# ysong1231/SimRank

Measured on AMD Instinct MI355X. Metric: simrank_iterations_per_sec, higher is better.
Workload: dtype f32

## Files before the change

simrank_amd/csrc/api.hip:

```cpp
#include <algorithm>
#include <chrono>
#include <cstring>
#include <mutex>
#include <unordered_map>
#include <string>
#include <thread>
#include <vector>

#include "common.h"

namespace simrank {

static thread_local char g_err[512] = "";

void set_error(const char* fmt, ...) {
    va_list ap;
    va_start(ap, fmt);
    vsnprintf(g_err, sizeof(g_err), fmt, ap);
    va_end(ap);
}

Tuning& tuning() {
    static Tuning t;
    return t;
// ... 67 lines not shown
            l.push_back((int32_t)rt);
        }
    }
    size_t longest = 0;
    for (const auto& l : lists) longest = std::max(longest, l.size() / 2);
    sym_map.assign(longest * 8 * 2, -1);
    for (size_t x = 0; x < 8; ++x)
        for (size_t k = 0; k < lists[x].size() / 2; ++k) {
            sym_map[2 * (8 * k + x)] = lists[x][2 * k];
            sym_map[2 * (8 * k + x) + 1] = lists[x][2 * k + 1];
        }
    return n_tiles;
}

void build_short_image(const int32_t* rowptr, const int32_t* col, const float* rowscale, int64_t n_rows,
                       const std::vector<int32_t>& tile_row0, int64_t n_tiles, int32_t width, ShortImage& out) {
    out = ShortImage();
    if ((width != 8 && width != 16) || n_tiles <= 0 || n_rows < 64) return;
    const int64_t groups = (n_tiles + 3) / 4;
    out.is_short.assign((size_t)groups, 0);
    for (int64_t k = 0; k < groups; ++k) {
        bool ok = true;
        for (int64_t t = 4 * k; ok && t < std::min<int64_t>(4 * k + 4, n_tiles); ++t) {
            const int64_t lo = tile_row0[(size_t)t], hi = tile_row0[(size_t)t + 1];
            ok = lo % 32 == 0 && hi == std::min<int64_t>(n_rows, lo + 32);
            for (int64_t a = lo; ok && a < hi; ++a) ok = rowptr[a + 1] - rowptr[a] <= width;
        }
        out.is_short[(size_t)k] = ok ? 1 : 0;
        out.groups += ok ? 1 : 0;
    }
    if (out.groups == 0) return;
    out.width = width;
    const size_t tiles_pad = (size_t)groups * 4;
    out.tiles.assign(tiles_pad * 2, 0);
    out.meta.assign(tiles_pad * 8 * 8, 0u);
    out.ids.assign(tiles_pad * 64 * (size_t)(width / 2), (uint16_t)0xFFFF);
    const int nc = width / 8;
    for (int64_t t = 0; t < n_tiles; ++t) {
        if (!out.is_short[(size_t)(t / 4)]) continue;
        const int32_t lo = tile_row0[(size_t)t];
        const int nrows = tile_row0[(size_t)t + 1] - lo;
        out.tiles[2 * (size_t)t] = lo;
        out.tiles[2 * (size_t)t + 1] = nrows;
        int order[32];
        for (int r = 0; r < nrows; ++r) order[r] = r;
        std::sort(order, order + nrows, [&](int x, int y) {
            const int32_t lx = rowptr[lo + x + 1] - rowptr[lo + x], ly = rowptr[lo + y + 1] - rowptr[lo + y];
            return lx != ly ? lx > ly : x > y;
        });
        for (int s = 0; s < nrows; ++s) {
            const int r = order[s], ps = s / 8, g = s % 8;
            const int32_t start = rowptr[lo + r], len = rowptr[lo + r + 1] - start;
            uint32_t* m = out.meta.data() + ((size_t)t * 8 + (size_t)g) * 8;
            std::memcpy(m + ps, rowscale + lo + r, 4);
            m[4] |= (uint32_t)len << (8 * ps);
            m[5] |= (uint32_t)r << (8 * ps);
            for (int32_t j = 0; j < len; ++j) {
                const int lane = 8 * g + (j & 7), c = j >> 3;
                out.ids[((size_t)t * 64 + (size_t)lane) * (size_t)(width / 2) + (size_t)(ps * nc + c)] = (uint16_t)col[start + j];
            }
        }
    }
}

namespace {
constexpr size_t kPoolMin = size_t(64) << 20;
constexpr size_t kSmallLimit = size_t(1) << 30;
constexpr int kSmallClasses = 4 * 40;
inline size_t small_class_bytes(int c) { return (size_t(4 + (c & 3)) << (c >> 2)) * 128; }
inline int small_class_of(size_t bytes) {
    int c = 0;
    while (small_class_bytes(c) < bytes) ++c;
    return c;
}
// ... 614 lines not shown
    int rc = up((void**)&g->rowptr, rowptr, size_t(n_rows + 1) * 4);
    if (!rc) rc = up((void**)&g->col, col, size_t(nnz) * 4);
    if (!rc && n_cols <= 65536 && nnz > 0) {
        std::vector<uint16_t> c16(col, col + nnz);
        rc = up((void**)&g->col16, c16.data(), size_t(nnz) * 2);
    }
    if (!rc) rc = up((void**)&g->rowscale, rowscale, size_t(n_rows) * 4);
    if (!rc) rc = up((void**)&g->t_rowptr, t_rowptr.data(), size_t(n_cols + 1) * 4);
    if (!rc) rc = up((void**)&g->t_col, t_col.data(), size_t(nnz) * 4);
    if (!rc) rc = up((void**)&g->t_pos, t_pos.data(), size_t(nnz) * 4);
    if (!rc && g->ev_hubs) rc = up((void**)&g->ev_hubidx, hubidx.data(), size_t(n_cols) * 4);
    if (!rc && g->n_tiles) rc = up((void**)&g->tile_row0, tile_row0.data(), tile_row0.size() * 4);
    if (!rc && g->sym_blocks) rc = up((void**)&g->sym_map, sym_map.data(), sym_map.size() * 4);
    if (!rc && g->sym_blocks && g->col16 && g->tun.leg2_short > 0) {
        ShortImage img;
        build_short_image(rowptr, col, rowscale, n_rows, tile_row0, g->n_tiles, (int32_t)g->tun.leg2_short, img);
        if (img.groups > 0) {
            for (size_t k = 0; k < sym_map.size() / 2; ++k)
                if (sym_map[2 * k] >= 0 && img.is_short[(size_t)sym_map[2 * k + 1]]) sym_map[2 * k + 1] |= 1 << 30;
            g->short_w = img.width;
            g->short_groups = img.groups;
            rc = up((void**)&g->sym_map_short, sym_map.data(), sym_map.size() * 4);
            if (!rc) rc = up((void**)&g->short_tiles, img.tiles.data(), img.tiles.size() * 4);
            if (!rc) rc = up((void**)&g->short_meta, img.meta.data(), img.meta.size() * 4);
            if (!rc) rc = up((void**)&g->short_ids, img.ids.data(), img.ids.size() * 2);
        }
    }
    if (!rc && after_base && *after_base) rc = (*after_base)(g);
    const double t_base = since();
    for (int i = 0; i < n_jobs; ++i) {
        jobs[i].th.join();
        if (timed) std::fprintf(stderr, "simrank_graph_create: builder %d took %.1f ms\n", i, jobs[i].ms);
        if (!rc && jobs[i].rc) {
            rc = jobs[i].rc;
// ... 172 lines not shown
        t.fuse_dens = value;
    } else if (!strcmp(key, "dense_cols")) {
        SR_REQUIRE(value >= 1 && value <= (1 << 20), "dense_cols must be >= 1");
        t.dense_cols = value;
    } else if (!strcmp(key, "restrict_support")) {
        SR_REQUIRE(value >= -1 && value <= 1, "restrict_support must be -1 (automatic), 0 or 1");
        t.restrict_support = value;
    } else if (!strcmp(key, "leg1_skip")) {
        t.leg1_skip = value ? 1 : 0;
    } else if (!strcmp(key, "leg1_order")) {
        SR_REQUIRE(value >= -1 && value <= 1, "leg1_order must be -1 (by the graph's size), 0 or 1");
        t.leg1_order = value;
    } else if (!strcmp(key, "leg2_short")) {
        SR_REQUIRE(value == 0 || value == 8 || value == 16, "leg2_short must be 0 (off), 8 or 16");
        t.leg2_short = value;
    } else {
        SR_REQUIRE(false, "unknown tuning key '%s'", key);
    }
    return SIMRANK_OK;
}

int simrank_get_tuning(const char* key, int64_t* value) {
    SR_REQUIRE(key && value, "NULL argument");
    const Tuning t = tuning_snapshot();
    if (!strcmp(key, "panel")) *value = t.panel;
    else if (!strcmp(key, "xcd_map")) *value = t.xcd_map;
    else if (!strcmp(key, "stream_nt")) *value = t.stream_nt;
    else if (!strcmp(key, "tile")) *value = t.tile;
    else if (!strcmp(key, "triangle")) *value = t.triangle;
    else if (!strcmp(key, "huge")) *value = t.huge;
// ... 18 lines not shown
    else if (!strcmp(key, "fuse_max_rows")) *value = t.fuse_max_rows;
    else if (!strcmp(key, "fuse_order")) *value = t.fuse_order;
    else if (!strcmp(key, "fuse_store")) *value = t.fuse_store;
    else if (!strcmp(key, "fuse_meta_nt")) *value = t.fuse_meta_nt;
    else if (!strcmp(key, "sym_desc")) *value = t.sym_desc;
    else if (!strcmp(key, "ids16")) *value = t.ids16;
    else if (!strcmp(key, "lean")) *value = t.lean;
    else if (!strcmp(key, "addr32")) *value = t.addr32;
    else if (!strcmp(key, "probe_flags")) *value = t.probe_flags;
    else if (!strcmp(key, "dense_terms")) *value = t.dense_terms;
    else if (!strcmp(key, "probe_mask")) *value = t.probe_mask;
    else if (!strcmp(key, "restrict_support")) *value = t.restrict_support;
    else if (!strcmp(key, "leg1_skip")) *value = t.leg1_skip;
    else if (!strcmp(key, "leg1_order")) *value = t.leg1_order;
    else if (!strcmp(key, "leg2_short")) *value = t.leg2_short;
    else SR_REQUIRE(false, "unknown tuning key '%s'", key);
    return SIMRANK_OK;
}

int simrank_graph_get(const simrank_graph* g, const char* key, int64_t* value) {
    SR_REQUIRE(g && key && value, "NULL argument");
    if (!strcmp(key, "fused_ids16")) *value = g->fused ? g->fused->ids16 : -1;
    else if (!strcmp(key, "gather_ids16")) *value = (g->col16 && g->tun.ids16) ? 1 : 0;
    else if (!strcmp(key, "leg2_short_groups")) *value = g->short_groups;
    else if (!strcmp(key, "leg2_short_taken")) *value = g->leg2_short_taken;
    else if (!strcmp(key, "ev_hubs")) *value = g->ev_hub_cols;
    else SR_REQUIRE(false, "unknown graph key '%s'", key);
    return SIMRANK_OK;
}

}
```

simrank_amd/csrc/biplan.hip:

```cpp
#include <algorithm>
#include <cstring>
#include <numeric>
#include <vector>

#include <chrono>
#include <string>
#include <thread>

#include "loop.h"
#include "side.h"

using simrank::side_t;

struct simrank_biplan {
    side_t s[2];
    unsigned long long* counters = nullptr;
    unsigned long long* host_counters[2][2] = {{nullptr, nullptr}, {nullptr, nullptr}};
    hipEvent_t counted[2] = {nullptr, nullptr};
    hipStream_t stream = nullptr;
    int32_t updates = 0;
    int32_t broadcast_error = 0;
    int32_t asym = 0;
    int32_t identity_leg1 = 1;
    int32_t at_identity = 0;
// ... 82 lines not shown
        if (rc) return rc;
    }
    lap("validated, ordered, both patterns renamed");
    const float* priors[2] = {opt->apriori1, opt->apriori2};
    const int64_t lds[2] = {opt->ld_apriori1, opt->ld_apriori2};
    const int64_t ns[2] = {n1, n2};
    const std::vector<int32_t>* ord = pp.ord;
    const std::vector<int32_t>* inv = pp.inv;
    simrank_biplan* p = new simrank_biplan;
    p->stream = as_stream(stream);
    p->asym = pp.asym ? 1 : 0;
    if (const char* e = std::getenv("SIMRANK_IDENTITY_LEG1")) p->identity_leg1 = (*e == '0') ? 0 : 1;
    auto fail = [&](int code) { simrank_biplan_destroy(p); return code; };
    {
        Tuning tw[2] = {tuning_snapshot(), Tuning()};
        tw[1] = tw[0];
        int rcs[2] = {SIMRANK_OK, SIMRANK_OK};
        std::string errs[2];
        for (int w = 0; w < 2; ++w) {
            side_t& a = p->s[w];
            side_shape(a, ns[w], ns[w ^ 1], false);
            a.coef = w == 0 ? opt->c1 : opt->c2;
            a.lbd = w == 0 ? opt->lbd1 : opt->lbd2;
            if (tw[w].fuse == 1 && ((tw[w].triangle && a.n >= 64) || p->asym) && a.k <= tw[w].fuse_max_rows &&
                (a.k_rows_pad + 1) * 128 < (int64_t(1) << 31))
                tw[w].dense_lazy = 1;
        }
        auto make = [&](int w) {
            side_t& a = p->s[w];
            rcs[w] = graph_create_with(tw[w], a.n, a.k, nnz, pp.rp[w].data(), pp.cl[w].data(), pp.rs[w].data(), &a.g);
// ... 182 lines not shown
```

simrank_amd/csrc/common.h:

```cpp
#pragma once
#include <hip/hip_runtime.h>

#include <cstdarg>
#include <atomic>
#include <cstdint>
#include <cstdio>
#include <cstdlib>
#include <cstring>
#include <functional>
#include <vector>

#include "simrank_hip.h"

namespace simrank {

void set_error(const char* fmt, ...);

#define SR_HIP(call)                                                                   \
    do {                                                                               \
        hipError_t e_ = (call);                                                        \
        if (e_ != hipSuccess) {                                                        \
            ::simrank::set_error("%s failed: %s (%s:%d)", #call, hipGetErrorString(e_), \
                                 __FILE__, __LINE__);                                  \
            return SIMRANK_ERR_HIP;                                                    \
// ... 14 lines not shown
    int64_t stream_nt = 1;
    int64_t tile = 0;
    int64_t huge = 512;
    int64_t triangle = 1;
    int64_t balance = 2;
    int64_t dense_min = 4;
    int64_t dense_cols = 128;
    int64_t dense_terms = 3;
    int64_t probe_mask = -1;
    int64_t probe_flags = 0;
    int64_t addr32 = 1;
    int64_t lean = 1;
    int64_t ids16 = 1;
    int64_t sym_desc = 1;
    int64_t leg2_short = 16;
    int64_t ev_tri = 1;
    int64_t ev_hub = 14;
    int64_t fuse = 1;
    int64_t fuse_min = 0;
    int64_t fuse_pays = -1;
    int64_t fuse_steps = -1;
    int64_t fuse_dens = 0;
    int64_t fuse_unit = 48;
    int64_t fuse_rows = 8192;
    int64_t fuse_store = 1;
    int64_t fuse_meta_nt = 0;
    int64_t fuse_order = 0;
    int64_t fuse_max_rows = 1 << 20;
    int64_t fuse_cap = 40000;
    int64_t fuse_wgs = 4;
// ... 188 lines not shown
#endif
struct DenseUse {
    const float* part = nullptr;
    int64_t ldp = 0;
    const int32_t* block_slab0 = nullptr;
    const int32_t* block_nslab = nullptr;
};
void free_dense_plan(simrank_dense_plan* p);
int build_dense_plan(simrank_graph* g, const int32_t* rowptr, const int32_t* col);
int launch_dense_tiles(const simrank_graph* g, const float* X, int64_t ldx, int64_t L, bool tri,
                       hipStream_t st, DenseUse* use);
int64_t build_tiles(const int32_t* rowptr, int64_t n_rows, int64_t nnz, int64_t balance,
                    std::vector<int32_t>& tile_row0, std::vector<int32_t>& sym_map, bool sym_descending);
struct ShortImage {
    int32_t width = 0, groups = 0;
    std::vector<uint8_t> is_short;
    std::vector<int32_t> tiles;
    std::vector<uint32_t> meta;
    std::vector<uint16_t> ids;
};
void build_short_image(const int32_t* rowptr, const int32_t* col, const float* rowscale, int64_t n_rows,
                       const std::vector<int32_t>& tile_row0, int64_t n_tiles, int32_t width, ShortImage& out);
}

struct simrank_graph {
    int64_t n_rows = 0, n_cols = 0, nnz = 0;
    int32_t* rowptr = nullptr;
    int32_t* col = nullptr;
    uint16_t* col16 = nullptr;
    float* rowscale = nullptr;
    int32_t* t_rowptr = nullptr;
    int32_t* t_col = nullptr;
    int32_t* t_pos = nullptr;
    int32_t* ev_hubidx = nullptr;
    int32_t ev_hubs = 0;
    int32_t ev_hub_cols = 0;
    uint8_t* ev_hub_image = nullptr;
    void* ev_hub_ready = nullptr;
    int32_t max_row_nnz = 0;
    int32_t* tile_row0 = nullptr;
    int32_t n_tiles = 0;
    int32_t* sym_map = nullptr;
    int32_t sym_blocks = 0;
    int32_t* sym_map_short = nullptr;
    uint32_t* short_ids = nullptr;
    uint32_t* short_meta = nullptr;
    int32_t* short_tiles = nullptr;
    int32_t short_w = 0, short_groups = 0;
    mutable int32_t leg2_short_taken = 0;
    simrank_dense_plan* dense = nullptr;
    simrank_fused_plan* fused = nullptr;
    std::atomic<int> fused_build{0};
#ifdef SIMRANK_EXPERIMENT_FUSED2
    simrank_fused2_plan* fused2 = nullptr;
#endif
    simrank::Tuning tun;
};
```

simrank_amd/csrc/shardplan.hip:

```cpp
#include <dlfcn.h>
#include <rccl/rccl.h>

#include <algorithm>
#include <chrono>
#include <condition_variable>
#include <cstdlib>
#include <cstring>
#include <deque>
#include <mutex>
#include <vector>

#include "common.h"
#include "loop.h"

static_assert(sizeof(ncclUniqueId) == SIMRANK_COMM_ID_BYTES, "RCCL's unique id is SIMRANK_COMM_ID_BYTES long");

namespace simrank {

struct Rccl {
    void* lib = nullptr;
    ncclResult_t (*GetUniqueId)(ncclUniqueId*) = nullptr;
    ncclResult_t (*CommInitRank)(ncclComm_t*, int, ncclUniqueId, int) = nullptr;
    ncclResult_t (*CommDestroy)(ncclComm_t) = nullptr;
    ncclResult_t (*GroupStart)() = nullptr;
// ... 876 lines not shown
    }
    p->ld = pitch(p->Lm, 4);
    p->ld_ev = pitch(p->Lm, 1);
    p->pad = row_pad(p->mb);
    p->send_ld = int64_t(P) * (p->mb + p->pad);
    p->recv_ld = std::max<int64_t>(1, p->Lm + p->pad);
    p->n_stages = in.stages > 0 ? in.stages : int32_t(std::max<int64_t>(1, std::min<int64_t>(4, ((k + P - 1) / P) / 2048)));
    p->ord = ord;
    auto fail = [&](int code) { simrank_shardplan_destroy(p); return code; };
    p->half = fp16 ? 1 : 0;
    p->rows_pad = (n + 7) / 8 * 8 + 8;
    p->rows_pad_t = (p->Lm + 7) / 8 * 8 + 8;
    int rc;
    {
        Tuning t = tuning_snapshot();
        if (fp16) t.fuse_unit = int64_t(1) << 20;
        rc = graph_create_with(t, n, k, in.nnz, in.pat->rp->data(), in.pat->cl->data(), in.pat->rs->data(), &p->g);
    }
    if (rc) return fail(rc);
    if (fp16 && !p->g->fused) {
        set_error("storage_fp16 needs the one-launch plan (tuning fuse = 1) and a graph that has one");
        return fail(SIMRANK_ERR_INVALID);
    }
#define SP_HIP(call)                                                                              \
    do {                                                                                          \
        hipError_t e_ = (call);                                                                   \
        if (e_ != hipSuccess) {                                                                   \
            set_error("%s failed: %s (%s:%d)", #call, hipGetErrorString(e_), __FILE__, __LINE__); \
            (void)hipGetLastError();                                                              \
            return fail(e_ == hipErrorOutOfMemory ? SIMRANK_ERR_ALLOC : SIMRANK_ERR_HIP);         \
// ... 708 lines not shown
```

simrank_amd/csrc/side.h:

```cpp
#pragma once
#include <cstring>
#include <vector>

#include "common.h"

namespace simrank {

constexpr float kHalfScale = 16384.0f;

#define SIDE_HIP(call)                                                                            \
    do {                                                                                          \
        hipError_t e_ = (call);                                                                   \
        if (e_ != hipSuccess) {                                                                   \
            set_error("%s failed: %s (%s:%d)", #call, hipGetErrorString(e_), __FILE__, __LINE__); \
            (void)hipGetLastError();                                                              \
            return e_ == hipErrorOutOfMemory ? SIMRANK_ERR_ALLOC : SIMRANK_ERR_HIP;               \
        }                                                                                         \
    } while (0)

struct side_t {
    int64_t n = 0, k = 0, rows_pad = 0, k_rows_pad = 0;
    size_t mat_bytes = 0, t_bytes = 0;
    simrank_graph* g = nullptr;
    float* S[2] = {nullptr, nullptr};
    float* Tt = nullptr;
    uint8_t* ev = nullptr;
    float* prior = nullptr;
    int32_t* inv = nullptr;
    int32_t* ord_dev = nullptr;
    std::vector<int32_t> ord;
    float coef = 0.8f, lbd = 0.f;
    int32_t restrict_support = 0;
    int32_t half = 0;
    int cur = 0;
    int32_t* first_block = nullptr;
    std::vector<int32_t> first_block_host;
    int64_t leg1_units = 0, leg1_skipped = 0;
    int64_t leg2_short_groups = 0;
    int64_t dead_units = -1;
};

inline size_t side_f32_bytes(const side_t& a) { return size_t((a.n + 31) / 32) * size_t(a.rows_pad) * 32 * sizeof(float); }

inline void side_shape(side_t& a, int64_t n, int64_t k, bool half) {
    a.n = n;
    a.k = k;
    a.half = half ? 1 : 0;
    a.rows_pad = (n + 7) / 8 * 8 + 8;
    a.k_rows_pad = (k + 7) / 8 * 8 + 8;
    const size_t panels = half ? size_t((n + 63) / 64) : size_t((n + 31) / 32);
    a.mat_bytes = panels * size_t(a.rows_pad) * 128;
    a.t_bytes = panels * size_t(a.k_rows_pad) * 128;
}
// ... 112 lines not shown
            a.leg1_skipped = a.dead_units;
        }
    }
    if (!rc) rc = stamp();
    if (rc) return rc;
    if (asym) {
        ep.symmetric = 0;
        ep.restrict_support = 0;
        rc = simrank_spmm_blocked(a.g, a.Tt, a.k_rows_pad, a.n, a.S[nx], a.rows_pad, 1, nullptr, st);
        if (!rc) rc = simrank_epilogue_apply_blocked(a.S[nx], a.S[nx], a.n, a.n, a.rows_pad, &ep, st);
    } else {
        rc = a.half ? simrank_spmm_blocked_h16(a.g, a.Tt, a.k_rows_pad, a.n, a.S[nx], a.rows_pad, 0, &ep, a.rows_pad, kHalfScale, st)
                    : simrank_spmm_blocked(a.g, a.Tt, a.k_rows_pad, a.n, a.S[nx], a.rows_pad, 0, &ep, st);
    }
    a.leg2_short_groups = (asym || a.half || rc) ? 0 : a.g->leg2_short_taken;
    if (!rc) rc = stamp();
    if (rc) return rc;
    SR_HIP(hipMemcpyAsync(host_slot, counters, sizeof(unsigned long long) * SIMRANK_CHANGED_SLOTS, hipMemcpyDeviceToHost, st));
    return SIMRANK_OK;
}

inline int side_f32(const side_t& a, hipStream_t st, const float** src, float** scratch) {
    *src = a.S[a.cur];
    *scratch = nullptr;
    if (!a.half) return SIMRANK_OK;
    SR_HIP(pool_hip_alloc((void**)scratch, side_f32_bytes(a)));
    *src = *scratch;
    return simrank_widen_blocked_h16(a.S[a.cur], a.rows_pad, *scratch, a.rows_pad, a.n, a.n, kHalfScale, st);
}

// ... 68 lines not shown
    }
    return SIMRANK_OK;
}

inline int side_get(const side_t& a, const char* key, int64_t* value) {
    if (!strcmp(key, "restrict_support")) *value = a.restrict_support;
    else if (!strcmp(key, "iterate")) *value = (int64_t)(uintptr_t)a.S[a.cur];
    else if (!strcmp(key, "iterate_layout")) *value = a.half ? 2 : 0;
    else if (!strcmp(key, "iterate_stride")) *value = a.rows_pad;
    else if (!strcmp(key, "iterate_rows") || !strcmp(key, "iterate_col_hi")) *value = a.n;
    else if (!strcmp(key, "iterate_col_lo")) *value = 0;
    else if (!strcmp(key, "ids")) *value = (int64_t)(uintptr_t)a.ord_dev;
    else if (!strcmp(key, "leg1_units")) *value = a.leg1_units;
    else if (!strcmp(key, "leg1_skipped")) *value = a.leg1_skipped;
    else if (!strcmp(key, "leg2_short_groups")) *value = a.leg2_short_groups;
    else if (!strcmp(key, "graph")) *value = (int64_t)(uintptr_t)a.g;
    else SR_REQUIRE(false, "unknown plan key '%s'", key);
    return SIMRANK_OK;
}

}
```

simrank_amd/csrc/spmm.hip:

```cpp
#include <algorithm>
#include <type_traits>

#include <mutex>

#include "common.h"

namespace simrank {

__device__ __forceinline__ int64_t imin(int64_t a, int64_t b) { return a < b ? a : b; }

__device__ __forceinline__ int64_t elem_at(int64_t r, int64_t c, int64_t ld, int64_t rows_pad) {
    return rows_pad ? ((c >> 5) * rows_pad + r) * 32 + (c & 31) : r * ld + c;
}

struct SpmmArgs {
    const int32_t* rowptr;
    const int32_t* col;
    const uint16_t* col16;
    int32_t blocked;
    int64_t x_rows_pad, y_rows_pad;
    int64_t x_span_bytes;
    int32_t x_sentinel;
    int32_t addr32;
    int32_t sh_rank, sh_mb;
// ... 38 lines not shown
    int64_t ld_ev;
    const float* ap;
    int64_t ld_ap;
    const float* prev;
    int64_t ld_prev;
    double eps;
    unsigned long long* n_changed;
    int64_t diag_col0;
    int32_t set_diag;
    int32_t count_any;
    int32_t restrict_support;
    const float* dpart;
    int64_t ldp;
    const int32_t* dslab0;
    const int32_t* dnslab;
};

template <int VEC>
__device__ __forceinline__ void vload(float (&d)[VEC], const float* p) {
    if constexpr (VEC == 4) {
        const float4 t = *reinterpret_cast<const float4*>(p);
        d[0] = t.x; d[1] = t.y; d[2] = t.z; d[3] = t.w;
    } else {
        d[0] = *p;
    }
}

template <int VEC>
__device__ __forceinline__ void vstore(float* p, const float (&d)[VEC]) {
    if constexpr (VEC == 4) {
// ... 651 lines not shown
                for (int i = 0; i < 4; ++i) t[i * (RT + 1)] = o[i];
            }
        }
        float* y = p.Y + a * p.ldy + colofs;
        if (p.probe & 2) {
        } else if (nvalid == 4) {
            if (p.nt) vstore_nt<4>(y, o); else vstore<4>(y, o);
        } else {
#pragma unroll
            for (int i = 0; i < 4; ++i)
                if (i < nvalid) y[i] = o[i];
        }
    }
}

constexpr int kShortFlag = 1 << 30;

__device__ __forceinline__ void short_group3(const SpmmArgs& p, const Src32& xs, float* tbuf_wave, int t, int panel, int lane,
                                             int64_t c0, int64_t mycol, int64_t colofs, bool col_active, bool check_prev,
                                             unsigned& changed) {
    constexpr int RT = 32, PW = 32;
    typedef unsigned v2u __attribute__((ext_vector_type(2)));
    typedef unsigned v4u __attribute__((ext_vector_type(4)));
    typedef float f4 __attribute__((ext_vector_type(4)));
    const int g = lane >> 3, q = lane & 7, gbase = lane & ~7;
    const int nc = p.short_w >> 3;
    const int row0 = p.short_tiles[2 * t];
    int nrows = p.short_tiles[2 * t + 1];
    const uint32_t* idp = p.short_ids + (size_t(t) * 64 + lane) * size_t(2 * nc);
    v4u idw = {0u, 0u, 0u, 0u};
    if (nc == 2) {
        idw = *reinterpret_cast<const v4u*>(idp);
    } else {
        const v2u w = *reinterpret_cast<const v2u*>(idp);
        idw.x = w.x;
        idw.y = w.y;
    }
    const uint32_t* meta = p.short_meta + (size_t(t) * 8 + g) * 8;
    const f4 scales = *reinterpret_cast<const f4*>(meta);
    const v2u lr = *reinterpret_cast<const v2u*>(meta + 4);
    if (row0 > c0) nrows = 0;
    const bool mirror = row0 < c0;
    if (nrows == 0) return;

    const __amdgpu_buffer_rsrc_t prd = __builtin_amdgcn_make_buffer_rsrc(
        const_cast<float*>(check_prev ? p.prev + int64_t(panel) * p.y_rows_pad * 32 : p.prev), 0,
        check_prev ? int(p.y_rows_pad * 128) : 0, 0x00020000);
    float old[4][4];
#pragma unroll
    for (int ps = 0; ps < 4; ++ps) {
        const int r = int((lr.y >> (8 * ps)) & 255u);
        const v4u w = __builtin_amdgcn_raw_buffer_load_b128(prd, (row0 + r) * 128 + q * 16, 0, 2);
        old[ps][0] = __uint_as_float(w.x); old[ps][1] = __uint_as_float(w.y);
        old[ps][2] = __uint_as_float(w.z); old[ps][3] = __uint_as_float(w.w);
    }
    const float dsum[4] = {0.f, 0.f, 0.f, 0.f};
    auto pass = [&](int ps, const float (&old_ps)[4], float sc) {
        if (8 * ps >= nrows) return;
        const int len = int((lr.x >> (8 * ps)) & 255u);
        const int r = int((lr.y >> (8 * ps)) & 255u);
        const int n = (p.probe & 1) ? 0 : __builtin_amdgcn_readfirstlane(len);
        float acc[4] = {0.f, 0.f, 0.f, 0.f};
#pragma unroll 1
        for (int k = 0; k < n; k += 8) {
            const int h = ps * nc + (k >> 3);
            const unsigned w01 = (h & 2) ? idw.y : idw.x, w23 = (h & 2) ? idw.w : idw.z;
            const int raw = int((((h & 4) ? w23 : w01) >> (16 * (h & 1))) & 0xFFFFu);
            const int iv = (k + q < len && !(p.probe & 8)) ? (raw & p.idx_mask) : xs.sent();
            gather_chunk<1>(xs, iv, gbase, min(8, n - k), 0, 0, acc);
        }
        if (8 * ps + g < nrows && col_active)
            emit_row3<kSym>(p, tbuf_wave, r, int64_t(row0) + r, q, mycol, colofs, sc, acc, dsum, changed, mirror, check_prev, old_ps);
    };
    pass(0, old[0], scales.x);
    pass(1, old[1], scales.y);
    pass(2, old[2], scales.z);
    pass(3, old[3], scales.w);

    if (mirror && !(p.probe & 2)) {
        __builtin_amdgcn_fence(__ATOMIC_RELEASE, "wavefront");
        __builtin_amdgcn_wave_barrier();
        __builtin_amdgcn_fence(__ATOMIC_ACQUIRE, "wavefront");
        const int cols_here = int(imin(PW, p.L - c0));
        float* base = p.Y + ((int64_t(row0 >> 5) * p.y_rows_pad) + c0) * 32;
        if (cols_here == PW && (nrows & 3) == 0) {
#pragma unroll
            for (int it = 0; it < PW * (RT / 4) / 64; ++it) {
                const int x = lane + it * 64;
                const int c = x >> 3;
                const int r4 = (x & 7) * 4;
                if (r4 < nrows) {
                    const float* tb = tbuf_wave + c * (RT + 1) + r4;
                    const float v4[4] = {tb[0], tb[1], tb[2], tb[3]};
                    float* dst = base + c * 32 + r4;
                    if (p.nt) vstore_nt<4>(dst, v4); else vstore<4>(dst, v4);
                }
            }
        } else {
            for (int x = lane; x < PW * RT; x += 64) {
                const int c = x >> 5;
                const int r = x & 31;
                if (c < cols_here && r < nrows) base[c * 32 + r] = tbuf_wave[c * (RT + 1) + r];
            }
        }
    }
}

#ifdef SIMRANK_STAMPS
__device__ unsigned long long g_stamps[16];
__device__ __forceinline__ unsigned long long stamp_now() {
    unsigned long long t;
    __builtin_amdgcn_sched_barrier(0);
    asm volatile("s_memtime %0\n\ts_waitcnt lgkmcnt(0)" : "=s"(t) :: "memory");
    __builtin_amdgcn_sched_barrier(0);
    return t;
}
#define STAMP(i)                                                          \
    do {                                                                  \
        const unsigned long long now_ = stamp_now();                      \
        if (lane == 0) atomicAdd(&g_stamps[i], now_ - stamp_prev);        \
        stamp_prev = now_;                                                \
    } while (0)
#else
#define STAMP(i) do {} while (0)
#endif

template <int MODE, bool IDS16, bool RESTRICT, bool DENSE, bool A32, bool SHORT = false>
#ifndef SIMRANK_LB_DELTA
#define SIMRANK_LB_DELTA 0
#endif
__global__ __launch_bounds__(256, (MODE == kTrans ? ((DENSE && !A32) ? 7 : 8) : (DENSE ? 5 : 6)) - SIMRANK_LB_DELTA)
void gather3_kernel(const SpmmArgs p) {
    constexpr bool TRANS = MODE == kTrans;
    constexpr bool TILE = MODE != kPlain;
    constexpr int PW = 32, RT = 32, LPR = 8;
    extern __shared__ __attribute__((aligned(16))) float smem[];
    if (p.probe & 32) return;

    const int lane = threadIdx.x & 63;
    const int wave = __builtin_amdgcn_readfirstlane(threadIdx.x >> 6);
#ifdef SIMRANK_STAMPS
    unsigned long long stamp_prev = stamp_now();
// ... 66 lines not shown
    const unsigned slot = ((blockIdx.x * 4u + unsigned(wave)) * 7u) % SIMRANK_CHANGED_SLOTS;
    if constexpr (!TRANS) {
        {
            typedef unsigned v2u __attribute__((ext_vector_type(2)));
            const bool watch = p.has_ep && p.prev && p.count_any;
            const __amdgpu_buffer_rsrc_t csrd = __builtin_amdgcn_make_buffer_rsrc(
                const_cast<unsigned long long*>(p.n_changed), 0, watch ? SIMRANK_CHANGED_SLOTS * 8 : 0, 0x00020000);
            const v2u w = __builtin_amdgcn_raw_buffer_load_b64(csrd, int(slot * 8u), 0, 16);
            seen = (unsigned long long)w.x | ((unsigned long long)w.y << 32);
        }
    }

    if constexpr (SHORT) {
        if (rt & kShortFlag) {
            const bool cp = p.has_ep && p.prev && __builtin_amdgcn_readfirstlane(int(seen != 0)) == 0;
            const int t = (rt & ~kShortFlag) * kWaves + wave;
            short_group3(p, xs, tbuf_wave, t, panel, lane, c0, mycol, colofs, col_active, cp, changed);
            STAMP(3);
            if (p.has_ep && p.prev) {
#pragma unroll
                for (int off = 32; off > 0; off >>= 1) changed += __shfl_down(changed, off);
                if (lane == 0 && changed) atomicAdd(p.n_changed + slot, (unsigned long long)changed);
            }
            return;
        }
    }

    int row0 = (rt * kWaves + wave) * RT;
    int nrows = int(imin(RT, p.M - row0));
    if (p.tile_row0) {
        const int t = rt * kWaves + wave;
        const int tc = __builtin_amdgcn_readfirstlane(max(0, min(t, p.n_tiles - 1)));
// ... 304 lines not shown
            }
        }
    }

    STAMP(5);
    if constexpr (!TRANS) {
        if (p.has_ep && p.prev) {
#pragma unroll
            for (int off = 32; off > 0; off >>= 1) changed += __shfl_down(changed, off);
            if (lane == 0 && changed) atomicAdd(p.n_changed + slot, (unsigned long long)changed);
        }
    }
}

template <int MODE>
static int launch_gather3(SpmmArgs a, hipStream_t st, int32_t* short_taken = nullptr) {
    constexpr int PW = 32, RT = 32;
    a.n_panels = int((a.L + PW - 1) / PW);
    if (MODE == kShard && a.sh_ntiles > 0) a.n_panels = a.sh_ntiles;
    const int64_t rows_per_block = int64_t(kWaves) * RT;
    a.row_tiles = int((a.M + rows_per_block - 1) / rows_per_block);
    if (MODE == kSym && !a.sym_map) a.tile_row0 = nullptr;
    if (a.tile_row0) a.row_tiles = (a.n_tiles + kWaves - 1) / kWaves;
    const int64_t panels_padded = a.xcd_map ? int64_t((a.n_panels + 7) / 8) * 8 : a.n_panels;
    int64_t grid = panels_padded * a.row_tiles;
    if constexpr (MODE == kSym) {
        const int64_t J = (a.n_panels + 7) / 8;
        grid = 8 * (J * J + J);
        if (a.tile_row0) grid = a.sym_blocks;
    }
    SR_REQUIRE(grid > 0 && grid < (int64_t(1) << 31), "grid of %lld blocks", (long long)grid);
    const size_t lds = sizeof(float) * ((MODE != kPlain ? size_t(kWaves) * PW * (RT + 1) : 0) +
                                        (a.has_huge ? 64 + size_t(kMaxHuge) * kWaves * PW : 0));
    const bool restricted = MODE != kTrans && a.has_ep && a.ev && a.restrict_support;
    const bool dense = a.dpart != nullptr;
    const dim3 gr((unsigned)grid), bl(256);
    const int64_t x_rows = a.blocked ? a.x_rows_pad : a.K;
    const int64_t span = a.blocked ? a.x_rows_pad * 128 : ((x_rows - 1) * a.ldx + a.ldx) * 4;
    const bool a32 = a.addr32 && (x_rows + 1) * a.ldx * 4 + 256 < (int64_t(1) << 31) &&
                     a.ldx * 4 < (int64_t(1) << 24) && x_rows < (int64_t(1) << 24) - 1;
    a.x_span_bytes = span;
    a.x_sentinel = (int32_t)x_rows;
    const bool take_short = MODE == kSym && a.sym_map_short && a.short_groups > 0 && a.tile_row0 && a32 && a.col16 &&
                            !restricted && !dense && a.blocked;
    if (!take_short) a.short_groups = 0;
    if (short_taken) *short_taken = a.short_groups;
    if constexpr (MODE == kSym) {
        if (take_short) {
            a.sym_map = a.sym_map_short;
            hipLaunchKernelGGL((gather3_kernel<kSym, true, false, false, true, true>), gr, bl, lds, st, a);
            SR_HIP(hipGetLastError());
            return SIMRANK_OK;
        }
    }
#define SR_LAUNCH3(IDS, RES, DEN) \
    do { if (a32) hipLaunchKernelGGL((gather3_kernel<MODE, IDS, RES, DEN, true>), gr, bl, lds, st, a); \
         else hipLaunchKernelGGL((gather3_kernel<MODE, IDS, RES, DEN, false>), gr, bl, lds, st, a); } while (0)
#define SR_LAUNCH3_IDS(RES, DEN) \
    do { if (a.col16) SR_LAUNCH3(true, RES, DEN); else SR_LAUNCH3(false, RES, DEN); } while (0)
    if constexpr (MODE != kTrans) {
        if (restricted) {
            if (dense) SR_LAUNCH3_IDS(true, true); else SR_LAUNCH3_IDS(true, false);
// ... 615 lines not shown
    a.M = g->n_rows;
    a.K = g->n_cols;
    a.tblock = (t_block <= 0 || t_block > g->n_rows) ? g->n_rows : t_block;
    a.tstride = (transpose_out && a.tblock == g->n_rows && ldy >= g->n_rows) ? ldy : 0;
    a.tpad = a.tstride ? 0 : t_pad;
    a.tvec = aligned16(Y) && (a.tstride ? a.tstride % 4 == 0
                                        : (a.tblock % 4 == 0 && a.tpad % 4 == 0 && g->n_rows % 4 == 0));
    a.xcd_map = (int)T.xcd_map;
    a.idx_mask = (int32_t)T.probe_mask;
    a.addr32 = (int32_t)T.addr32;
    a.probe = (int32_t)T.probe_flags;
    bool vec_ok = aligned16(X) && ldx % 4 == 0;
    if (!transpose_out) vec_ok = vec_ok && aligned16(Y) && ldy % 4 == 0;
    hipStream_t st = as_stream(stream);
    if (ep) {
        if (!(sk && sk->dry)) g->leg2_short_taken = 0;
        a.has_ep = 1;
        a.coef = ep->coef;
        a.lbd = ep->lbd;
        a.ev = ep->evidence;
        a.ld_ev = ep->ld_evidence;
        a.ap = ep->apriori;
        a.ld_ap = ep->ld_apriori;
        a.prev = ep->previous;
        a.ld_prev = ep->ld_previous;
        a.eps = ep->eps;
        a.n_changed = ep->n_changed;
        a.diag_col0 = ep->diag_col0;
        a.set_diag = ep->set_diag;
        a.restrict_support = ep->restrict_support;
        a.count_any = ep->count_any;
// ... 59 lines not shown
    }
    if (T.balance) {
        const int32_t* tr0 = dp ? dp->r_tile_row0 : g->tile_row0;
        if (tr0) {
            a.tile_row0 = tr0;
            a.n_tiles = dp ? dp->r_n_tiles : g->n_tiles;
            a.sym_map = dp ? dp->r_sym_map : g->sym_map;
            a.sym_blocks = dp ? dp->r_sym_blocks : g->sym_blocks;
            if (!dp && g->sym_map_short) {
                a.sym_map_short = g->sym_map_short;
                a.short_ids = g->short_ids;
                a.short_meta = g->short_meta;
                a.short_tiles = g->short_tiles;
                a.short_w = g->short_w;
                a.short_groups = g->short_groups;
            }
        }
    }
    if (!vec_ok) {
        SR_REQUIRE(!blocked, "panel-blocked operands must be 16-byte aligned");
        return transpose_out ? launch_spmm<1, 32, kTrans, 32>(a, st)
                             : launch_spmm<1, 32, kPlain, 32>(a, st);
    }
    const bool lean_ok = T.lean && tile == 32 && ldx / 4 < (int64_t(1) << 24) &&
                         g->n_cols < (int64_t(1) << 24) && g->n_cols * (ldx / 4) < (int64_t(1) << 32) &&
                         g->n_rows < (int64_t(1) << 30);
    if (blocked) {
        SR_REQUIRE(lean_ok && (T.panel == 0 || T.panel == 32),
                   "panel-blocked operands need the lean kernel (tile 32, panel 32, < 2^24 rows)");
        if (want_sym) return launch_gather3<kSym>(a, st, &g->leg2_short_taken);
        return transpose_out ? launch_gather3<kTrans>(a, st) : launch_gather3<kPlain>(a, st);
    }
    if (lean_ok && want_sym) {
        a.tblock = g->n_rows;
        a.tstride = ldy;
        return launch_gather3<kSym>(a, st);
    }
    if (lean_ok && transpose_out && (T.panel == 0 || T.panel == 32))
        return launch_gather3<kTrans>(a, st);
    if (lean_ok && !transpose_out && (T.panel == 0 || T.panel == 32))
        return launch_gather3<kPlain>(a, st);
#define SR_TILE_SWITCH(LPR, TR)                                             \
    switch (tile) {                                                         \
        case 16: return launch_spmm<4, LPR, TR, 16>(a, st);                 \
        case 32: return launch_spmm<4, LPR, TR, 32>(a, st);                 \
// ... 461 lines not shown
```

Measured before the change: 149.5.

## Add narrow class for short tile groups with rows up to eight entries

Splits the short-row image into two sections. Groups whose rows all hold at most eight neighbours get a compact 8-wide id record, loaded as one 64-bit read per lane, and are flagged in the symmetric map so the kernel dispatches a one-chunk specialised path. The aim is to cut id bytes loaded and padded gather work for very sparse rows. The cost is a new kernel variant with a runtime branch per group and more code size and register pressure. It is on by default but turned off for biplan and shard plans.

```diff
diff --git a/simrank_amd/csrc/api.hip b/simrank_amd/csrc/api.hip
--- a/simrank_amd/csrc/api.hip
+++ b/simrank_amd/csrc/api.hip
@@ -105,34 +105,53 @@
 }
 
 void build_short_image(const int32_t* rowptr, const int32_t* col, const float* rowscale, int64_t n_rows,
-                       const std::vector<int32_t>& tile_row0, int64_t n_tiles, int32_t width, ShortImage& out) {
+                       const std::vector<int32_t>& tile_row0, int64_t n_tiles, int32_t width, ShortImage& out, bool narrow) {
     out = ShortImage();
     if ((width != 8 && width != 16) || n_tiles <= 0 || n_rows < 64) return;
     const int64_t groups = (n_tiles + 3) / 4;
     out.is_short.assign((size_t)groups, 0);
+    out.is_narrow.assign((size_t)groups, 0);
     for (int64_t k = 0; k < groups; ++k) {
         bool ok = true;
+        int32_t longest = 0;
         for (int64_t t = 4 * k; ok && t < std::min<int64_t>(4 * k + 4, n_tiles); ++t) {
             const int64_t lo = tile_row0[(size_t)t], hi = tile_row0[(size_t)t + 1];
             ok = lo % 32 == 0 && hi == std::min<int64_t>(n_rows, lo + 32);
-            for (int64_t a = lo; ok && a < hi; ++a) ok = rowptr[a + 1] - rowptr[a] <= width;
+            for (int64_t a = lo; ok && a < hi; ++a) {
+                longest = std::max(longest, rowptr[a + 1] - rowptr[a]);
+                ok = rowptr[a + 1] - rowptr[a] <= width;
+            }
         }
         out.is_short[(size_t)k] = ok ? 1 : 0;
         out.groups += ok ? 1 : 0;
-    }
-    if (out.groups == 0) return;
+        if (ok && narrow && longest <= 8) {
+            out.is_narrow[(size_t)k] = 1;
+            out.narrow_groups += 1;
+        }
+    }
+    if (out.groups == 0) {
+        out.is_narrow.clear();
+        return;
+    }
     out.width = width;
+    out.narrow = narrow ? 1 : 0;
     const size_t tiles_pad = (size_t)groups * 4;
     out.tiles.assign(tiles_pad * 2, 0);
     out.meta.assign(tiles_pad * 8 * 8, 0u);
-    out.ids.assign(tiles_pad * 64 * (size_t)(width / 2), (uint16_t)0xFFFF);
-    const int nc = width / 8;
+    const size_t wide_tiles = narrow ? (size_t)(out.groups - out.narrow_groups) * 4 : tiles_pad;
+    out.ids.assign(wide_tiles * 64 * (size_t)(width / 2), (uint16_t)0xFFFF);
+    out.ids_narrow.assign((size_t)out.narrow_groups * 4 * 64 * 4, (uint16_t)0xFFFF);
+    size_t next_wide = 0, next_narrow = 0;
     for (int64_t t = 0; t < n_tiles; ++t) {
         if (!out.is_short[(size_t)(t / 4)]) continue;
+        const bool nar = out.is_narrow[(size_t)(t / 4)] != 0;
+        const size_t slot = !narrow ? (size_t)t : nar ? next_narrow++ : next_wide++;
+        const int w = nar ? 8 : width, nc = w / 8;
+        uint16_t* rec = (nar ? out.ids_narrow.data() : out.ids.data()) + slot * 64 * (size_t)(w / 2);
         const int32_t lo = tile_row0[(size_t)t];
         const int nrows = tile_row0[(size_t)t + 1] - lo;
         out.tiles[2 * (size_t)t] = lo;
-        out.tiles[2 * (size_t)t + 1] = nrows;
+        out.tiles[2 * (size_t)t + 1] = nrows | (narrow ? (int32_t)(slot << 8) : 0);
         int order[32];
         for (int r = 0; r < nrows; ++r) order[r] = r;
         std::sort(order, order + nrows, [&](int x, int y) {
@@ -148,7 +167,7 @@
             m[5] |= (uint32_t)r << (8 * ps);
             for (int32_t j = 0; j < len; ++j) {
                 const int lane = 8 * g + (j & 7), c = j >> 3;
-                out.ids[((size_t)t * 64 + (size_t)lane) * (size_t)(width / 2) + (size_t)(ps * nc + c)] = (uint16_t)col[start + j];
+                rec[(size_t)lane * (size_t)(w / 2) + (size_t)(ps * nc + c)] = (uint16_t)col[start + j];
             }
         }
     }
@@ -793,10 +812,17 @@
     if (!rc && g->sym_blocks) rc = up((void**)&g->sym_map, sym_map.data(), sym_map.size() * 4);
     if (!rc && g->sym_blocks && g->col16 && g->tun.leg2_short > 0) {
         ShortImage img;
-        build_short_image(rowptr, col, rowscale, n_rows, tile_row0, g->n_tiles, (int32_t)g->tun.leg2_short, img);
-        if (img.groups > 0) {
+        const bool narrow = g->tun.leg2_narrow != 0;
+        build_short_image(rowptr, col, rowscale, n_rows, tile_row0, g->n_tiles, (int32_t)g->tun.leg2_short, img, narrow);
+        if (img.groups > 0 && narrow) {
+            g->short_narrow_ofs = (int32_t)(img.ids.size() / 2);
+            g->narrow_groups = img.narrow_groups;
+            img.ids.insert(img.ids.end(), img.ids_narrow.begin(), img.ids_narrow.end());
+        }
+        if (!rc && img.groups > 0) {
             for (size_t k = 0; k < sym_map.size() / 2; ++k)
-                if (sym_map[2 * k] >= 0 && img.is_short[(size_t)sym_map[2 * k + 1]]) sym_map[2 * k + 1] |= 1 << 30;
+                if (sym_map[2 * k] >= 0 && img.is_short[(size_t)sym_map[2 * k + 1]])
+                    sym_map[2 * k + 1] |= kShortFlag | (img.is_narrow[(size_t)sym_map[2 * k + 1]] ? kNarrowFlag : 0);
             g->short_w = img.width;
             g->short_groups = img.groups;
             rc = up((void**)&g->sym_map_short, sym_map.data(), sym_map.size() * 4);
@@ -999,6 +1025,8 @@
     } else if (!strcmp(key, "leg2_short")) {
         SR_REQUIRE(value == 0 || value == 8 || value == 16, "leg2_short must be 0 (off), 8 or 16");
         t.leg2_short = value;
+    } else if (!strcmp(key, "leg2_narrow")) {
+        t.leg2_narrow = value ? 1 : 0;
     } else {
         SR_REQUIRE(false, "unknown tuning key '%s'", key);
     }
@@ -1047,6 +1075,7 @@
     else if (!strcmp(key, "leg1_skip")) *value = t.leg1_skip;
     else if (!strcmp(key, "leg1_order")) *value = t.leg1_order;
     else if (!strcmp(key, "leg2_short")) *value = t.leg2_short;
+    else if (!strcmp(key, "leg2_narrow")) *value = t.leg2_narrow;
     else SR_REQUIRE(false, "unknown tuning key '%s'", key);
     return SIMRANK_OK;
 }
@@ -1057,6 +1086,7 @@
     else if (!strcmp(key, "gather_ids16")) *value = (g->col16 && g->tun.ids16) ? 1 : 0;
     else if (!strcmp(key, "leg2_short_groups")) *value = g->short_groups;
     else if (!strcmp(key, "leg2_short_taken")) *value = g->leg2_short_taken;
+    else if (!strcmp(key, "leg2_narrow_groups")) *value = g->narrow_groups;
     else if (!strcmp(key, "ev_hubs")) *value = g->ev_hub_cols;
     else SR_REQUIRE(false, "unknown graph key '%s'", key);
     return SIMRANK_OK;
diff --git a/simrank_amd/csrc/biplan.hip b/simrank_amd/csrc/biplan.hip
--- a/simrank_amd/csrc/biplan.hip
+++ b/simrank_amd/csrc/biplan.hip
@@ -120,6 +120,7 @@
     auto fail = [&](int code) { simrank_biplan_destroy(p); return code; };
     {
         Tuning tw[2] = {tuning_snapshot(), Tuning()};
+        tw[0].leg2_narrow = 0;
         tw[1] = tw[0];
         int rcs[2] = {SIMRANK_OK, SIMRANK_OK};
         std::string errs[2];
diff --git a/simrank_amd/csrc/common.h b/simrank_amd/csrc/common.h
--- a/simrank_amd/csrc/common.h
+++ b/simrank_amd/csrc/common.h
@@ -52,6 +52,7 @@
     int64_t ids16 = 1;
     int64_t sym_desc = 1;
     int64_t leg2_short = 16;
+    int64_t leg2_narrow = 1;
     int64_t ev_tri = 1;
     int64_t ev_hub = 14;
     int64_t fuse = 1;
@@ -270,13 +271,18 @@
                     std::vector<int32_t>& tile_row0, std::vector<int32_t>& sym_map, bool sym_descending);
 struct ShortImage {
     int32_t width = 0, groups = 0;
+    int32_t narrow = 0, narrow_groups = 0;
     std::vector<uint8_t> is_short;
+    std::vector<uint8_t> is_narrow;
     std::vector<int32_t> tiles;
     std::vector<uint32_t> meta;
     std::vector<uint16_t> ids;
+    std::vector<uint16_t> ids_narrow;
 };
 void build_short_image(const int32_t* rowptr, const int32_t* col, const float* rowscale, int64_t n_rows,
-                       const std::vector<int32_t>& tile_row0, int64_t n_tiles, int32_t width, ShortImage& out);
+                       const std::vector<int32_t>& tile_row0, int64_t n_tiles, int32_t width, ShortImage& out,
+                       bool narrow = false);
+constexpr int32_t kShortFlag = 1 << 30, kNarrowFlag = 1 << 29;
 }
 
 struct simrank_graph {
@@ -303,7 +309,9 @@
     uint32_t* short_meta = nullptr;
     int32_t* short_tiles = nullptr;
     int32_t short_w = 0, short_groups = 0;
+    int32_t short_narrow_ofs = -1, narrow_groups = 0;
     mutable int32_t leg2_short_taken = 0;
+    mutable int32_t leg2_narrow_taken = 0;
     simrank_dense_plan* dense = nullptr;
     simrank_fused_plan* fused = nullptr;
     std::atomic<int> fused_build{0};
diff --git a/simrank_amd/csrc/shardplan.hip b/simrank_amd/csrc/shardplan.hip
--- a/simrank_amd/csrc/shardplan.hip
+++ b/simrank_amd/csrc/shardplan.hip
@@ -914,6 +914,7 @@
     int rc;
     {
         Tuning t = tuning_snapshot();
+        t.leg2_narrow = 0;
         if (fp16) t.fuse_unit = int64_t(1) << 20;
         rc = graph_create_with(t, n, k, in.nnz, in.pat->rp->data(), in.pat->cl->data(), in.pat->rs->data(), &p->g);
     }
diff --git a/simrank_amd/csrc/side.h b/simrank_amd/csrc/side.h
--- a/simrank_amd/csrc/side.h
+++ b/simrank_amd/csrc/side.h
@@ -37,6 +37,7 @@
     std::vector<int32_t> first_block_host;
     int64_t leg1_units = 0, leg1_skipped = 0;
     int64_t leg2_short_groups = 0;
+    int64_t leg2_narrow_groups = 0;
     int64_t dead_units = -1;
 };
 
@@ -179,6 +180,7 @@
                     : simrank_spmm_blocked(a.g, a.Tt, a.k_rows_pad, a.n, a.S[nx], a.rows_pad, 0, &ep, st);
     }
     a.leg2_short_groups = (asym || a.half || rc) ? 0 : a.g->leg2_short_taken;
+    a.leg2_narrow_groups = (asym || a.half || rc) ? 0 : a.g->leg2_narrow_taken;
     if (!rc) rc = stamp();
     if (rc) return rc;
     SR_HIP(hipMemcpyAsync(host_slot, counters, sizeof(unsigned long long) * SIMRANK_CHANGED_SLOTS, hipMemcpyDeviceToHost, st));
@@ -277,6 +279,7 @@
     else if (!strcmp(key, "leg1_units")) *value = a.leg1_units;
     else if (!strcmp(key, "leg1_skipped")) *value = a.leg1_skipped;
     else if (!strcmp(key, "leg2_short_groups")) *value = a.leg2_short_groups;
+    else if (!strcmp(key, "leg2_narrow_groups")) *value = a.leg2_narrow_groups;
     else if (!strcmp(key, "graph")) *value = (int64_t)(uintptr_t)a.g;
     else SR_REQUIRE(false, "unknown plan key '%s'", key);
     return SIMRANK_OK;
diff --git a/simrank_amd/csrc/spmm.hip b/simrank_amd/csrc/spmm.hip
--- a/simrank_amd/csrc/spmm.hip
+++ b/simrank_amd/csrc/spmm.hip
@@ -76,6 +76,8 @@
     int64_t ldp;
     const int32_t* dslab0;
     const int32_t* dnslab;
+    int32_t short_narrow_ofs;
+    int32_t narrow_groups;
 };
 
 template <int VEC>
@@ -757,20 +759,93 @@
     }
 }
 
-constexpr int kShortFlag = 1 << 30;
-
+
+__device__ __forceinline__ void short_mirror3(const SpmmArgs& p, const float* tbuf_wave, int row0, int nrows, int lane, int64_t c0) {
+    constexpr int RT = 32, PW = 32;
+    __builtin_amdgcn_fence(__ATOMIC_RELEASE, "wavefront");
+    __builtin_amdgcn_wave_barrier();
+    __builtin_amdgcn_fence(__ATOMIC_ACQUIRE, "wavefront");
+    const int cols_here = int(imin(PW, p.L - c0));
+    float* base = p.Y + ((int64_t(row0 >> 5) * p.y_rows_pad) + c0) * 32;
+    if (cols_here == PW && (nrows & 3) == 0) {
+#pragma unroll
+        for (int it = 0; it < PW * (RT / 4) / 64; ++it) {
+            const int x = lane + it * 64;
+            const int c = x >> 3;
+            const int r4 = (x & 7) * 4;
+            if (r4 < nrows) {
+                const float* tb = tbuf_wave + c * (RT + 1) + r4;
+                const float v4[4] = {tb[0], tb[1], tb[2], tb[3]};
+                float* dst = base + c * 32 + r4;
+                if (p.nt) vstore_nt<4>(dst, v4); else vstore<4>(dst, v4);
+            }
+        }
+    } else {
+        for (int x = lane; x < PW * RT; x += 64) {
+            const int c = x >> 5;
+            const int r = x & 31;
+            if (c < cols_here && r < nrows) base[c * 32 + r] = tbuf_wave[c * (RT + 1) + r];
+        }
+    }
+}
+
+template <int NC, bool CLASSES>
 __device__ __forceinline__ void short_group3(const SpmmArgs& p, const Src32& xs, float* tbuf_wave, int t, int panel, int lane,
                                              int64_t c0, int64_t mycol, int64_t colofs, bool col_active, bool check_prev,
                                              unsigned& changed) {
-    constexpr int RT = 32, PW = 32;
     typedef unsigned v2u __attribute__((ext_vector_type(2)));
     typedef unsigned v4u __attribute__((ext_vector_type(4)));
     typedef float f4 __attribute__((ext_vector_type(4)));
+    static_assert(NC == 2 || CLASSES, "the narrow class exists in the two-section image only");
     const int g = lane >> 3, q = lane & 7, gbase = lane & ~7;
+    const int row0 = p.short_tiles[2 * t];
+    const int rec = p.short_tiles[2 * t + 1];
+    int nrows = CLASSES ? (rec & 255) : rec;
+    const int slot = CLASSES ? (rec >> 8) : t;
+    const uint32_t* meta = p.short_meta + (size_t(t) * 8 + g) * 8;
+    const float dsum[4] = {0.f, 0.f, 0.f, 0.f};
+    if constexpr (NC == 1) {
+        const v2u idw = *reinterpret_cast<const v2u*>(p.short_ids + size_t(p.short_narrow_ofs) + (size_t(slot) * 64 + lane) * 2);
+        const f4 scales = *reinterpret_cast<const f4*>(meta);
+        const v2u lr = *reinterpret_cast<const v2u*>(meta + 4);
+        if (row0 > c0) nrows = 0;
+        const bool mirror = row0 < c0;
+        if (nrows == 0) return;
+        const __amdgpu_buffer_rsrc_t prd = __builtin_amdgcn_make_buffer_rsrc(
+            const_cast<float*>(check_prev ? p.prev + int64_t(panel) * p.y_rows_pad * 32 : p.prev), 0,
+            check_prev ? int(p.y_rows_pad * 128) : 0, 0x00020000);
+        float old[4][4];
+        auto request = [&](int ps, float (&o)[4]) {
+            const int r = int((lr.y >> (8 * ps)) & 255u);
+            const v4u w = __builtin_amdgcn_raw_buffer_load_b128(prd, (row0 + r) * 128 + q * 16, 0, 2);
+            o[0] = __uint_as_float(w.x); o[1] = __uint_as_float(w.y);
+            o[2] = __uint_as_float(w.z); o[3] = __uint_as_float(w.w);
+        };
+        request(0, old[0]);
+        request(1, old[1]);
+        request(2, old[2]);
+        request(3, old[3]);
+        auto pass = [&](int ps, float (&old_ps)[4], float sc) {
+            if (8 * ps >= nrows) return;
+            const int len = int((lr.x >> (8 * ps)) & 255u);
+            const int r = int((lr.y >> (8 * ps)) & 255u);
+            const int n = (p.probe & 1) ? 0 : __builtin_amdgcn_readfirstlane(len);
+            const int raw = int((((ps & 2) ? idw.y : idw.x) >> (16 * (ps & 1))) & 0xFFFFu);
+            const int iv = (q < len && !(p.probe & 8)) ? (raw & p.idx_mask) : xs.sent();
+            float acc[4] = {0.f, 0.f, 0.f, 0.f};
+            gather_chunk<1>(xs, iv, gbase, n, 0, 0, acc);
+            if (8 * ps + g < nrows && col_active)
+                emit_row3<kSym>(p, tbuf_wave, r, int64_t(row0) + r, q, mycol, colofs, sc, acc, dsum, changed, mirror, check_prev, old_ps);
+        };
+        pass(0, old[0], scales.x);
+        pass(1, old[1], scales.y);
+        pass(2, old[2], scales.z);
+        pass(3, old[3], scales.w);
+        if (mirror && !(p.probe & 2)) short_mirror3(p, tbuf_wave, row0, nrows, lane, c0);
+        return;
+    }
     const int nc = p.short_w >> 3;
-    const int row0 = p.short_tiles[2 * t];
-    int nrows = p.short_tiles[2 * t + 1];
-    const uint32_t* idp = p.short_ids + (size_t(t) * 64 + lane) * size_t(2 * nc);
+    const uint32_t* idp = p.short_ids + (size_t(slot) * 64 + lane) * size_t(2 * nc);
     v4u idw = {0u, 0u, 0u, 0u};
     if (nc == 2) {
         idw = *reinterpret_cast<const v4u*>(idp);
@@ -779,7 +854,6 @@
         idw.x = w.x;
         idw.y = w.y;
     }
-    const uint32_t* meta = p.short_meta + (size_t(t) * 8 + g) * 8;
     const f4 scales = *reinterpret_cast<const f4*>(meta);
     const v2u lr = *reinterpret_cast<const v2u*>(meta + 4);
     if (row0 > c0) nrows = 0;
@@ -797,7 +871,6 @@
         old[ps][0] = __uint_as_float(w.x); old[ps][1] = __uint_as_float(w.y);
         old[ps][2] = __uint_as_float(w.z); old[ps][3] = __uint_as_float(w.w);
     }
-    const float dsum[4] = {0.f, 0.f, 0.f, 0.f};
     auto pass = [&](int ps, const float (&old_ps)[4], float sc) {
         if (8 * ps >= nrows) return;
         const int len = int((lr.x >> (8 * ps)) & 255u);
@@ -820,33 +893,7 @@
     pass(2, old[2], scales.z);
     pass(3, old[3], scales.w);
 
-    if (mirror && !(p.probe & 2)) {
-        __builtin_amdgcn_fence(__ATOMIC_RELEASE, "wavefront");
-        __builtin_amdgcn_wave_barrier();
-        __builtin_amdgcn_fence(__ATOMIC_ACQUIRE, "wavefront");
-        const int cols_here = int(imin(PW, p.L - c0));
-        float* base = p.Y + ((int64_t(row0 >> 5) * p.y_rows_pad) + c0) * 32;
-        if (cols_here == PW && (nrows & 3) == 0) {
-#pragma unroll
-            for (int it = 0; it < PW * (RT / 4) / 64; ++it) {
-                const int x = lane + it * 64;
-                const int c = x >> 3;
-                const int r4 = (x & 7) * 4;
-                if (r4 < nrows) {
-                    const float* tb = tbuf_wave + c * (RT + 1) + r4;
-                    const float v4[4] = {tb[0], tb[1], tb[2], tb[3]};
-                    float* dst = base + c * 32 + r4;
-                    if (p.nt) vstore_nt<4>(dst, v4); else vstore<4>(dst, v4);
-                }
-            }
-        } else {
-            for (int x = lane; x < PW * RT; x += 64) {
-                const int c = x >> 5;
-                const int r = x & 31;
-                if (c < cols_here && r < nrows) base[c * 32 + r] = tbuf_wave[c * (RT + 1) + r];
-            }
-        }
-    }
+    if (mirror && !(p.probe & 2)) short_mirror3(p, tbuf_wave, row0, nrows, lane, c0);
 }
 
 #ifdef SIMRANK_STAMPS
@@ -868,7 +915,7 @@
 #define STAMP(i) do {} while (0)
 #endif
 
-template <int MODE, bool IDS16, bool RESTRICT, bool DENSE, bool A32, bool SHORT = false>
+template <int MODE, bool IDS16, bool RESTRICT, bool DENSE, bool A32, bool SHORT = false, bool CLASSES = false>
 #ifndef SIMRANK_LB_DELTA
 #define SIMRANK_LB_DELTA 0
 #endif
@@ -965,8 +1012,13 @@
     if constexpr (SHORT) {
         if (rt & kShortFlag) {
             const bool cp = p.has_ep && p.prev && __builtin_amdgcn_readfirstlane(int(seen != 0)) == 0;
-            const int t = (rt & ~kShortFlag) * kWaves + wave;
-            short_group3(p, xs, tbuf_wave, t, panel, lane, c0, mycol, colofs, col_active, cp, changed);
+            const int t = (rt & ~(kShortFlag | kNarrowFlag)) * kWaves + wave;
+            if constexpr (CLASSES) {
+                if (rt & kNarrowFlag) short_group3<1, true>(p, xs, tbuf_wave, t, panel, lane, c0, mycol, colofs, col_active, cp, changed);
+                else short_group3<2, true>(p, xs, tbuf_wave, t, panel, lane, c0, mycol, colofs, col_active, cp, changed);
+            } else {
+                short_group3<2, false>(p, xs, tbuf_wave, t, panel, lane, c0, mycol, colofs, col_active, cp, changed);
+            }
             STAMP(3);
             if (p.has_ep && p.prev) {
 #pragma unroll
@@ -1301,7 +1353,7 @@
 }
 
 template <int MODE>
-static int launch_gather3(SpmmArgs a, hipStream_t st, int32_t* short_taken = nullptr) {
+static int launch_gather3(SpmmArgs a, hipStream_t st, int32_t* short_taken = nullptr, int32_t* narrow_taken = nullptr) {
     constexpr int PW = 32, RT = 32;
     a.n_panels = int((a.L + PW - 1) / PW);
     if (MODE == kShard && a.sh_ntiles > 0) a.n_panels = a.sh_ntiles;
@@ -1332,7 +1384,14 @@
                             !restricted && !dense && a.blocked;
     if (!take_short) a.short_groups = 0;
     if (short_taken) *short_taken = a.short_groups;
+    if (narrow_taken) *narrow_taken = (take_short && a.short_narrow_ofs >= 0) ? a.narrow_groups : 0;
     if constexpr (MODE == kSym) {
+        if (take_short && a.short_narrow_ofs >= 0) {
+            a.sym_map = a.sym_map_short;
+            hipLaunchKernelGGL((gather3_kernel<kSym, true, false, false, true, true, true>), gr, bl, lds, st, a);
+            SR_HIP(hipGetLastError());
+            return SIMRANK_OK;
+        }
         if (take_short) {
             a.sym_map = a.sym_map_short;
             hipLaunchKernelGGL((gather3_kernel<kSym, true, false, false, true, true>), gr, bl, lds, st, a);
@@ -1978,7 +2037,7 @@
     if (!transpose_out) vec_ok = vec_ok && aligned16(Y) && ldy % 4 == 0;
     hipStream_t st = as_stream(stream);
     if (ep) {
-        if (!(sk && sk->dry)) g->leg2_short_taken = 0;
+        if (!(sk && sk->dry)) g->leg2_short_taken = g->leg2_narrow_taken = 0;
         a.has_ep = 1;
         a.coef = ep->coef;
         a.lbd = ep->lbd;
@@ -2068,6 +2127,8 @@
                 a.short_tiles = g->short_tiles;
                 a.short_w = g->short_w;
                 a.short_groups = g->short_groups;
+                a.short_narrow_ofs = g->short_narrow_ofs;
+                a.narrow_groups = g->narrow_groups;
             }
         }
     }
@@ -2082,7 +2143,7 @@
     if (blocked) {
         SR_REQUIRE(lean_ok && (T.panel == 0 || T.panel == 32),
                    "panel-blocked operands need the lean kernel (tile 32, panel 32, < 2^24 rows)");
-        if (want_sym) return launch_gather3<kSym>(a, st, &g->leg2_short_taken);
+        if (want_sym) return launch_gather3<kSym>(a, st, &g->leg2_short_taken, &g->leg2_narrow_taken);
         return transpose_out ? launch_gather3<kTrans>(a, st) : launch_gather3<kPlain>(a, st);
     }
     if (lean_ok && want_sym) {
```

Result: no change. 149.9 (median of 6 runs) (+0.3%).
